# johannesulf/TabCorr

Measured on AMD Instinct MI355X. Metric: predict_calls_per_sec, higher is better.
Workload: dtype f64; 1 GPU; BASELINE configs[1]: Zheng07 predict(), synthetic auto table 50 mass bins x {cen,sat} (G=100, P=5050), 19 rp bins, n_gauss_prim=10, batch of 10000 draws per GPU per step, draws and results resident in HBM; n_tables=1, gather=none, gather_payload=ngal + xi (160 B per draw), gather_every_steps=32, lanes=4, rccl_ranks=0

## Files before the change

include/tabcorr_amd_testing.h:

```cpp
#ifndef TABCORR_AMD_TESTING_H
#define TABCORR_AMD_TESTING_H

#include "tabcorr_amd.h"

#ifdef __cplusplus
extern "C" {
#endif

int tc_debug_fastmath(int kind, int64_t n, const double* x, double* y);
int tc_debug_fastmath_device(int kind, int64_t n, const double* x, double* y);

int tc_debug_grad_operand(int n_bins, int n_r, const double* packed, double* dense);

int tc_debug_grad_lds(int kernel, int n_params, int n_bins, int n_central, int n_r, int n_dim,
                      int chi2, int64_t* bytes);

int tc_debug_leauthaud11_node_grad(const double* theta, int modulate, int64_t n,
                                   const double* mass, double* log_mstar, double* n_cen,
                                   double* dn_cen, double* n_sat, double* dn_sat);

int tc_debug_central_series(int n_gauss, double log_min, double log_max, double dist_index,
                            int64_t n, const double* log_m_min, const double* sigma,
                            double* series, double* nodes, int32_t* terms);

int tc_debug_satellite_series(int n_gauss, double log_min, double log_max, double dist_index,
                              int64_t n, const double* log_m0, const double* log_m1,
                              const double* alpha, double* series, double* nodes,
                              int32_t* terms);

int tc_plan_debug(int mode, int n_bins, const uint8_t* is_central, int n_chunks,
                  int64_t* n_entries, int32_t* entry_pair, int32_t* entry_chunk,
                  int32_t* entry_class);

int tc_debug_quad_schedule(int n_bins, int n_central, int by_type, int n_tiles, int n_rtiles,
                           int n_tables, int separate, int max_waves, int min_units,
                           int order ,
                           int* n_waves, int* n_runs, int* n_slabs, int64_t* units_min,
                           int64_t* units_max);
int tc_debug_triangle_parts(int n_rb, int n_parts, int32_t* rb0, int32_t* cb0, int32_t* count);
int tc_debug_node_groups(int n_bins, int n_central, const double* log_min,
                         const double* log_max, int32_t* begin, int32_t* member,
                         int* n_groups, int* n_central_groups);
int tc_debug_fused_form(int n_bins, int n_central, int n_r, int n_cus, int grouped,
                        int64_t n_draws, int n_gauss, unsigned flags, unsigned call,
                        const int* options, const int* measured_forms, const float* measured_us,
                        int* waves, int* draws, int* lds_bytes);
int tc_debug_pair_plan(const double* boxsize, double reach_xy, double reach_z,
                       int64_t n_points, int n_bin, int n_labels, int32_t* cells,
                       int32_t* neighbours, int32_t* labels_per_block, int32_t* n_blocks,
                       int64_t* lds_bytes);
int tc_debug_quad_emulate(int n_bins, int n_r, const double* tpcf_matrix,
                          const uint8_t* is_central, int by_type, int separate,
                          const double* densities, int64_t ldb, int64_t n_draws,
                          int max_waves, int min_units, int order, double* out);

int tc_debug_trace(tc_table* table, uint64_t* out, int64_t capacity, int64_t* n_blocks);
int tc_debug_wave_trace(tc_table* table, uint64_t* out, int64_t capacity,
                        int64_t* n_waves);
int tc_debug_resident_ticks(tc_table* table, uint64_t* out, int64_t capacity, int64_t* n_blocks);
int tc_debug_ensemble_stamps(tc_table* table, uint64_t* out);
#ifdef __cplusplus
}
// ... 4 lines not shown
```

tabcorr_amd/_lib.py:

```python

import ctypes
import os

import numpy as np

HERE = os.path.dirname(os.path.abspath(__file__))
LIBRARY = os.path.join(HERE, 'libtabcorr_hip.so')

TC_OK = 0
TC_ERR_INVALID = 1
TC_ERR_HIP = 2
TC_ERR_UNSUPPORTED = 3
TC_ERR_RCCL = 4

MODE = {'auto': 0, 'cross': 1}
DTYPE_F64 = 0
DTYPE_F32 = 1

FLAG_SEPARATE_GAL_TYPE = 1
FLAG_MODULATE_WITH_CENOCC = 2
FLAG_ASSEMBIAS = 4
FLAG_LEAUTHAUD11 = 16

UNIQUE_ID_BYTES = 128
# ... 19 lines not shown
    'tc_memcpy_d2h': [ctypes.c_void_p, ctypes.c_void_p, ctypes.c_size_t],
    'tc_host_alloc': [c_void_pp, ctypes.c_size_t],
    'tc_host_free': [ctypes.c_void_p],
    'tc_host_register': [ctypes.c_void_p, ctypes.c_size_t],
    'tc_host_unregister': [ctypes.c_void_p],
    'tc_host_is_pinned': [ctypes.c_void_p, ctypes.c_size_t, c_int_p],
    'tc_gauss_legendre': [ctypes.c_int, c_double_p, c_double_p],
    'tc_debug_fastmath': [ctypes.c_int, ctypes.c_int64, c_double_p,
                          c_double_p],
    'tc_debug_fastmath_device': [ctypes.c_int, ctypes.c_int64, c_double_p,
                                 c_double_p],
    'tc_debug_grad_operand': [ctypes.c_int, ctypes.c_int, c_double_p, c_double_p],
    'tc_debug_grad_lds': [ctypes.c_int] * 7 + [c_int64_p],
    'tc_debug_leauthaud11_node_grad': [c_double_p, ctypes.c_int, ctypes.c_int64, c_double_p,
                                       c_double_p, c_double_p, c_double_p, c_double_p,
                                       c_double_p],
    'tc_pair_indices': [ctypes.c_int, c_int32_p, c_int32_p, c_int32_p],
    'tc_spline_interpolation_matrix': [ctypes.c_int, c_double_p, c_double_p],
    'tc_spline_weights': [ctypes.c_int, c_double_p, c_double_p, ctypes.c_double, c_double_p,
                          c_double_p, c_int_p],
    'tc_plan_debug': [ctypes.c_int, ctypes.c_int, c_uint8_p, ctypes.c_int,
                      c_int64_p, c_int32_p, c_int32_p, c_int32_p],
    'tc_debug_triangle_parts': [ctypes.c_int, ctypes.c_int, c_int_p, c_int_p, c_int_p],
    'tc_debug_central_series': [ctypes.c_int, ctypes.c_double, ctypes.c_double, ctypes.c_double,
                                ctypes.c_int64, c_double_p, c_double_p, c_double_p, c_double_p,
                                c_int32_p],
    'tc_debug_satellite_series': [ctypes.c_int, ctypes.c_double, ctypes.c_double,
                                  ctypes.c_double, ctypes.c_int64, c_double_p, c_double_p,
                                  c_double_p, c_double_p, c_double_p, c_int32_p],
    'tc_debug_node_groups': [ctypes.c_int, ctypes.c_int, c_double_p, c_double_p,
                             c_int32_p, c_int32_p, c_int_p, c_int_p],
    'tc_debug_quad_schedule': [ctypes.c_int] * 10 + [c_int_p, c_int_p, c_int_p,
                                                     c_int64_p, c_int64_p],
    'tc_debug_fused_form': [ctypes.c_int] * 5 + [ctypes.c_int64, ctypes.c_int, ctypes.c_uint,
                                                 ctypes.c_uint, c_int_p, c_int_p,
                                                 c_float_p, c_int_p, c_int_p,
                                                 c_int_p],
    'tc_debug_pair_plan': [c_double_p, ctypes.c_double, ctypes.c_double, ctypes.c_int64,
                           ctypes.c_int, ctypes.c_int, c_int32_p, c_int32_p, c_int32_p,
                           c_int32_p, c_int64_p],
    'tc_debug_quad_emulate': [ctypes.c_int, ctypes.c_int, c_double_p, c_uint8_p,
                              ctypes.c_int, ctypes.c_int, c_double_p,
                              ctypes.c_int64, ctypes.c_int64, ctypes.c_int,
                              ctypes.c_int, ctypes.c_int, c_double_p],
    'tc_table_create': [
        ctypes.c_int, ctypes.c_int, ctypes.c_int, ctypes.c_int64,
# ... 239 lines not shown

_lib = None


class TabCorrHipError(RuntimeError):
    """The HIP backend failed (no device, launch error, RCCL error)."""


def load():
    global _lib
    if _lib is not None:
        return _lib
    library = os.environ.get('TABCORR_AMD_LIBRARY') or LIBRARY
    if not os.path.exists(library):
        raise TabCorrHipError(
            'libtabcorr_hip.so is missing: build it with '
            '`python -m tabcorr_amd.build` (needs hipcc). There is no CPU '
            'fallback.')
    mode = os.RTLD_NOW | os.RTLD_LOCAL | getattr(os, 'RTLD_DEEPBIND', 0)
    lib = ctypes.CDLL(library, mode=mode)
    lib.tc_last_error.restype = ctypes.c_char_p
    lib.tc_last_error.argtypes = []
    for name, argtypes in SIGNATURES.items():
        function = getattr(lib, name)
        function.restype = ctypes.c_int
        function.argtypes = argtypes
    _lib = lib
    return lib


def check(status):
    if status == TC_OK:
        return
    message = load().tc_last_error().decode(errors='replace')
    if status == TC_ERR_INVALID:
        raise ValueError(message)
    if status == TC_ERR_UNSUPPORTED:
        raise NotImplementedError(message)
    raise TabCorrHipError(message)


def as_double_p(array):
    try:
        return ctypes.byref(ctypes.c_double.from_buffer(array))
    except (TypeError, ValueError, BufferError):
        return array.ctypes.data_as(c_double_p)
# ... 36 lines not shown
```

tabcorr_amd/csrc/hostmath.cpp:

```cpp
#include "hostmath.h"
#include "fastmath.h"
#include "kernel_args.h"
#include "series.h"

#include <algorithm>
#include <atomic>
#include <cmath>
#include <cstring>
#include <map>
#include <numeric>
#include <tuple>
#include <thread>

namespace tc {

void gauss_legendre(int n, std::vector<double>& x, std::vector<double>& w) {
  x.assign(n, 0.0);
  w.assign(n, 0.0);
  const long double pi = 3.141592653589793238462643383279502884L;
  for (int i = 0; i < (n + 1) / 2; ++i) {
    long double z = cosl(pi * (i + 0.75L) / (n + 0.5L));
    long double dp = 1.0L;
    for (int iter = 0; iter < 100; ++iter) {
      long double p0 = 1.0L, p1 = z;
      for (int k = 2; k <= n; ++k) {
        long double p2 = ((2 * k - 1) * z * p1 - (k - 1) * p0) / k;
        p0 = p1;
        p1 = p2;
      }
      if (n == 0) p1 = 1.0L;
      dp = n * (z * p1 - p0) / (z * z - 1.0L);
// ... 690 lines not shown
    plan.block_begin[(size_t)block + 1] = (int32_t)plan.merges.size();
  }
  schedule.n_slabs = next_slab;
  const std::vector<int32_t> renumbered =
      number_slabs_by_group(slab_group, schedule.n_groups, schedule.group_begin);
  for (QuadRun& run : schedule.runs)
    if (run.slab >= 0) run.slab = renumbered[run.slab];
  for (QuadMerge& m : plan.merges) m.slab = renumbered[m.slab];
}

void triangle_parts(int n_rb, int n_parts, int32_t* rb0, int32_t* cb0, int32_t* count) {
  const int64_t n_units = (int64_t)n_rb * (n_rb + 1) / 2;
  for (int part = 0; part < n_parts; ++part) {
    const int64_t begin = n_units * part / n_parts, end = n_units * (part + 1) / n_parts;
    int64_t rb = (int64_t)((std::sqrt(8.0 * (double)begin + 1.0) - 1.0) / 2.0);
    while ((rb + 1) * (rb + 2) / 2 <= begin) ++rb;
    while (rb * (rb + 1) / 2 > begin) --rb;
    rb0[part] = (int32_t)rb;
    cb0[part] = (int32_t)(begin - rb * (rb + 1) / 2);
    count[part] = (int32_t)(end - begin);
  }
}

QuadTiling quad_tiling(int n_r) {
  QuadTiling tiling;
  tiling.n_rtiles = (n_r + 19) / 20;
  tiling.r_per_tile = (n_r + tiling.n_rtiles - 1) / tiling.n_rtiles;
  tiling.n_u = (tiling.r_per_tile + 3) / 4;
  return tiling;
}


int fused_dens_rows(const QuadLayout& layout) {
  int rows = 0;
  for (const QuadComp& comp : layout.comps)
    rows = std::max(rows, std::max(comp.i_bin0 + 4 * comp.n_rb, comp.j_bin0 + 4 * comp.n_cb));
  return (rows + 3) / 4 * 4;
}

int fused_lds_bytes(int dens_rows, int waves, int draws) {
  return (std::max(dens_rows * draws, fused_slot_doubles(waves, draws)) +
          fused_scratch_doubles(waves)) * 8;
}

FusedForm choose_fused_form(const FusedQuery& q) {
  const FusedForm three_kernels{};
// ... 579 lines not shown
```

tabcorr_amd/csrc/hostmath.h:

```cpp
#pragma once

#include <cstdint>
#include <string>
#include <vector>

namespace tc {

void gauss_legendre(int n, std::vector<double>& x, std::vector<double>& w);

inline int64_t packed_index(int64_t i, int64_t j) {
  return i >= j ? i * (i + 1) / 2 + j : j * (j + 1) / 2 + i;
}

bool spline_interpolation_matrix(int n, const double* xp, std::vector<double>& a);

struct Segment {
  int32_t component;
  int32_t rectangular;
  int32_t i_lo, i_hi;
  int32_t j_lo, j_hi;
  int64_t q_begin;
  int64_t n_real;
};

// ... 105 lines not shown
constexpr int kQuadUnitParts = 8;
void build_quad_schedule(const QuadLayout& layout, int n_tiles, int n_rtiles, int n_tables,
                         bool separate, int max_waves, int min_units_per_wave,
                         QuadSchedule& out, int order = kQuadTileMajor);

struct QuadMerge {
  int32_t slab;
  int32_t first_slot;
  int32_t count;
  int32_t pad;
};
struct QuadMergePlan {
  int waves_per_block = 0;
  int n_blocks = 0;
  int lds_slots = 0;
  std::vector<int32_t> block_begin;
  std::vector<QuadMerge> merges;
};
void merge_quad_schedule(const QuadLayout& layout, int n_rtiles, bool separate,
                         int waves_per_block, int max_slots, QuadSchedule& schedule,
                         QuadMergePlan& plan);

void triangle_parts(int n_rb, int n_parts, int32_t* rb0, int32_t* cb0, int32_t* count);

struct QuadTiling {
  int n_rtiles = 1;
  int r_per_tile = 0;
  int n_u = 0;
};
QuadTiling quad_tiling(int n_r);


struct AutoChoice {
  static constexpr int kSizes = 9;
  static constexpr int64_t size(int i) { return (int64_t)256 << i; }
  int form[kSizes] = {};
  float us[kSizes][3] = {};
  int form_for(int64_t n_draws) const {
    if (n_draws <= size(0)) return form[0];
    if (n_draws >= size(kSizes - 1)) return form[kSizes - 1];
    int i = 0;
    while (size(i + 1) < n_draws) ++i;
    const double w = (double)(n_draws - size(i)) / (double)(size(i + 1) - size(i));
    static const int shape[3] = {0, 64, 32};
    int best = 0;
    double best_us = (1.0 - w) * us[i][0] + w * us[i + 1][0];
// ... 102 lines not shown
```

tabcorr_amd/csrc/internal.h:

```cpp
#pragma once

#include <hip/hip_runtime.h>
#include <hip/hip_ext.h>

#include <algorithm>
#include <chrono>
#include <cmath>
#include <cstdarg>
#include <cstdio>
#include <cstdlib>
#include <cstring>
#include <functional>
#include <map>
#include <memory>
#include <string>
#include <utility>
#include <vector>

#include "../../include/tabcorr_amd.h"
#include "../../include/tabcorr_amd_testing.h"
#include "fastmath.h"
#include "grad.h"
#include "vjp.h"
#include "hostmath.h"
// ... 222 lines not shown
  int poll_done = 1;
  int quad_waves = 0;
  int quad_waves_f32 = 3;
  int quad_merge = 1;
  int quad_order = -1;
  int prio_occ = 2, prio_contract = 1, prio_finalize = 3;
  int finalize_threads = 0;
  int finalize_row_blocks = 0;
  int occ_splits = 0;
  int occ_per_cu = 4;
  int n_groups = 0, n_waves = 0, lds_min = 0, min_chunk_entries = 32;
  int k_splits = 0;
  int trace = 0;
  int autotune_after = 0;
  int sync_chunks = 0;
  int sync_form = 32;
  int sync_stagger = 10;
  int sync_direct_out = 2;
  int async_direct_in = 1;
  int async_direct_out = 2;
  int series = -1;
  int cross_defer = 1;
  int fused_defer = 2;
  int fused_sat_cap = 6;
  int cross_wide_min_draws = 4096;
  int cross_target = 160;
  int resident_aperture = 1;
  int cross_min_draws = 192;
  int fused = 1;
  int fused_min_draws = 0;
  int fused_max_draws = 30720;
  int fused_waves = 0;
  int fused_draws = 0;
  int fused_spread = 1, fused_spread_min = 8192, fused_spread_rounds = 1;
  int prio_fused = 1, prio_fused_occ = 2, prio_fused_out = 3;
  int deterministic = 0;
  int skip_occ = 0, skip_finalize = 0;
  void load() {
    fused = env_int("TC_FUSED", fused);
    fused_min_draws = env_int("TC_FUSED_MIN_DRAWS", fused_min_draws);
    fused_max_draws = env_int("TC_FUSED_MAX_DRAWS", fused_max_draws);
    prio_fused = env_int("TC_PRIO_FUSED", prio_fused);
    prio_fused_occ = env_int("TC_PRIO_FUSED_OCC", prio_fused_occ);
    prio_fused_out = env_int("TC_PRIO_FUSED_OUT", prio_fused_out);
    lanes = env_int("TC_LANES", lanes);
    pipeline = env_int("TC_PIPELINE", pipeline);
// ... 41 lines not shown
  std::vector<double> n_h, log_min, log_max, percentile, dist_index;

  void* d_table = nullptr;
  size_t table_bytes = 0;
  void* d_n_h = nullptr;
  void* d_percentile = nullptr;
  void* d_perm = nullptr;
  tc::NodeGroups node_groups;
  void* d_group_begin = nullptr;
  void* d_group_member = nullptr;
  void* d_group_n_h = nullptr;
  void* d_group_percentile = nullptr;
  bool grouped = false;
  void* d_math_table = nullptr;
  void* d_pos_ij = nullptr;
  void* d_pos_off = nullptr;
  std::vector<double> cross_host;
  tc::host::CrossFused cross_fused, cross_fused_wide;
  tc::host::GradTable grad;
  std::vector<hipEvent_t> chunk_events;
  bool quad = false;
  tc::QuadTiling quad_tiling;
  tc::host::QuadTable quad_by_type, quad_total;
  int n_cus = 256;
  int n_xcds = 8;
  tc::host::Tuning tuning;
  std::map<unsigned, AutoChoice> autotuned;
  std::map<unsigned, int> pipelined_calls;
  bool autotuning = false;
  std::map<int, tc::host::Quadrature> quadrature;
  std::map<std::pair<int, int>, std::unique_ptr<tc::host::DeviceChunking>> chunkings;
  std::map<int64_t, tc::host::DeviceChunking*> choices;

  struct Lane {
    hipStream_t stream = nullptr;
    hipEvent_t finished = nullptr;
    tc::host::DeviceBuffer nbuf, ngal2, partial;
    tc::host::DeviceBuffer nbuf32;
    tc::host::DeviceBuffer xi;
    tc::host::DeviceBuffer in_theta, out;
    tc::host::DeviceBuffer cross_counters;
    int ngal_parts = 1;
  };
  static constexpr int kMaxLanes = 8;
  Lane lanes[kMaxLanes];
  int n_lanes = 2;
// ... 258 lines not shown
```

tabcorr_amd/csrc/kernel_args.h:

```cpp
#pragma once

#include <cstdint>

#include "hostmath.h"

namespace tc {

constexpr int kLanes = 64;
constexpr unsigned kFlagSeparate = 1u;
constexpr unsigned kFlagModulate = 2u;
constexpr unsigned kFlagAssembias = 4u;
constexpr int kOccWaves = 4;
constexpr int kF32Block = 8;
constexpr int kF64Block = 8;
constexpr int kF32Tile = 32;
constexpr int kFinalizeRows = 32;
constexpr int kMaxInterpDim = 8;
constexpr int kMaxInterpAxis = 32;

struct GroupArgs {
  const int32_t* begin;
  const int32_t* member;
  const double* log_m;
  const double* m;
// ... 194 lines not shown
struct FinalizeQuadArgs {
  const void* partial;
  const int32_t* group_begin;
  const double* ngal_part;
  int n_ngal_parts;
  int n_rtiles;
  int r_per_tile;
  int rt;
  int groups_per_rtile;
  int n_comp;
  int n_r;
  int mode;
  int priority;
  int64_t ldb;
  int64_t n_draws;
  double* ngal;
  double* xi;
  const double* chi2_data;
  double* chi2;
};

constexpr int kFusedWaves = 8;
constexpr int kFusedMaxParts = 8;
constexpr int kMathTableDoubles = 2306;
constexpr int fused_slot_doubles(int waves, int draws = 64) {
  return waves * 4 * kQuadMaxU * (draws == 40 ? 40 : kQuadTile);
}
constexpr int fused_scratch_doubles(int waves) { return kMathTableDoubles + 2 * waves * kLanes; }

struct FusedArgs {
  const double* theta;
  int n_theta;
  int n_bins;
  int n_central;
  int n_gauss;
  int dens_rows;
  int part_rb0[kFusedMaxParts];
  int part_cb0[kFusedMaxParts];
  int part_count[kFusedMaxParts];
  int part_triangular[kFusedMaxParts];
  int part_n_cb[kFusedMaxParts];
  int part_i_row0[kFusedMaxParts];
  int part_j_row0[kFusedMaxParts];
  int part_unit_base[kFusedMaxParts];
  int separate;
  int n_r;
  int priority;
  int64_t n_draws;
  const double* log_m;
  const double* m;
  const double* weight;
  const double* n_h;
  const double* percentile;
  double split;
  const double* math_table;
  const void* table;
  uint32_t table_bytes;
  double* ngal;
  double* xi;
  const double* chi2_data;
  double* chi2;
  int n_groups;
  int n_central_groups;
  GroupArgs group;
  const double* series;
  const int32_t* series_thr;
  const double* sat_series;
// ... 106 lines not shown
```

tabcorr_amd/csrc/kernels.hip.h:

```cpp
#pragma once

#include <hip/hip_runtime.h>

#include <cstdint>
#include <utility>

#include "epilogue.h"
#include "fastmath.h"
#include "fused_walk.h"
#include "hostmath.h"
#include "kernel_args.h"
#include "series.h"
#include "spline.h"

#ifdef TC_DEVELOPER_KNOBS
#define TC_TRACE(pointer) ((pointer) != nullptr)
#else
#define TC_TRACE(pointer) false
#endif

namespace tc {

static_assert(sizeof(QuadRun) == 32 && sizeof(QuadCompArgs) == 32, "read as 8 x int32");

// ... 1885 lines not shown
  static_assert(!LEAUTHAUD || (NGAUSS == 0 && !ASSEMBIAS), "Leauthaud11: any n_gauss, undecorated");
  constexpr int UP = (U + 1) / 2;
  extern __shared__ __attribute__((aligned(16))) double fused_lds[];
  constexpr int kSlotDoubles = fused_slot_doubles(W, DL);
  const int region_b = a.dens_rows * DL > kSlotDoubles ? a.dens_rows * DL : kSlotDoubles;
  double* dens = fused_lds;
  double* table = fused_lds + region_b;
  double(*red)[W][kLanes] = (double(*)[W][kLanes])(table + fm::kTableDoubles);
  const fm::Consts kc = fm::make_consts();
#ifdef TC_DEVELOPER_KNOBS
  const int skip = (a.priority >> 8) & 3;
  const int n_bins_occ = (skip & 1) ? 0 : a.n_bins;
  unsigned long long* const stamps =
      ((a.priority >> 10) & 1) && a.chi2 == nullptr ? (unsigned long long*)a.chi2_data : nullptr;
  auto wave_stamp = [&](int which) {
    if (stamps != nullptr && (threadIdx.x & 63) == 0 && W == 8 && ((threadIdx.x >> 6) & 3) == 0)
      stamps[blockIdx.x * 32 + 16 + 8 * (threadIdx.x >> 8) + which] =
          __builtin_amdgcn_s_memrealtime();
  };
  auto stamp = [&](int which) {
    if (stamps != nullptr && threadIdx.x == 0)
      stamps[blockIdx.x * 32 + which] = __builtin_amdgcn_s_memrealtime();
  };
  if (skip & 1)
    for (int idx = threadIdx.x; idx < a.n_bins * DL; idx += blockDim.x) fused_lds[idx] = 1e-3;
#else
  constexpr int skip = 0;
  const int n_bins_occ = a.n_bins;
  auto stamp = [](int) {};
  auto wave_stamp = [](int) {};
#endif
  stamp(0);
  set_priority((a.priority >> 2) & 3);
  const int lane = threadIdx.x & 63;
  const int wave = __builtin_amdgcn_readfirstlane(threadIdx.x >> 6);
  const int n_gauss = NGAUSS > 0 ? NGAUSS : a.n_gauss;
  {
    typedef double __attribute__((ext_vector_type(2))) double2v;
    const int hi = fm::kTableDoubles / 2;
    const double2v* src = (const double2v*)a.math_table;
    double2v* dst = (double2v*)table;
    for (int i = threadIdx.x; i < hi; i += blockDim.x) dst[i] = src[i];
  }
  for (int idx = a.n_bins * DL + threadIdx.x; idx < a.dens_rows * DL; idx += blockDim.x)
    dens[idx] = 0.0;
  __syncthreads();
  stamp(1);

  const int draw = DL != 32 ? lane : (lane & 31);
  const int half = DL != 32 ? 0 : (lane >> 5);
  const bool live = DL != 40 || lane < 40;
  auto dens_at = [&](int row, int d) -> double& {
    return dens[DL == 40 ? dens40(row, d) : row * DL + d];
// ... 179 lines not shown
    stamp(3);
    red[0][wave][lane] = sum_cen;
    red[1][wave][lane] = sum_sat;
    __syncthreads();
    stamp(4);
    double n_cen = 0.0, n_sat = 0.0;
#pragma unroll
    for (int w = 0; w < W; ++w) {
      n_cen += red[0][w][lane];
      n_sat += red[1][w][lane];
    }
    const double total = (skip & 1) ? 1.0 : n_cen + n_sat;
    norm = total * total;
    if (wave == 0 && half == 0 && live && b0 < a.n_draws) {
      if (a.separate) {
        a.ngal[2 * b0] = n_cen;
        a.ngal[2 * b0 + 1] = n_sat;
      } else {
        a.ngal[b0] = total;
      }
    }
  }

  set_priority(a.priority & 3);
  const int c = lane & 15, kq = lane >> 4;
  double F[UP][2][2];
  constexpr int UA = DL == 40 ? (U > 3 ? 3 : U) : 1, UB = DL == 40 && U > 3 ? U - 3 : 1;
  double F40a[UA][10], F40b[UB][10];
  int slot = wave;
  if (DL == 40) {
    const int part = wave;
    const unsigned off_a = ((lane & 0x30) | ((lane & 3) << 2) | ((lane >> 2) & 3)) * 16;
    const double* dens_b = dens + (a.part_j_row0[part] + (lane >> 4)) * 40 + (lane & 3) * 10;
    const double* dens_e = dens + (a.part_i_row0[part] + (lane >> 4)) * 40 + (lane & 3) * 10;
    const __amdgpu_buffer_rsrc_t rs_t =
        __builtin_amdgcn_make_buffer_rsrc((void*)a.table, 0, a.table_bytes, kBufferFlags);
    const int rb = a.part_rb0[part], cb = a.part_cb0[part], count = a.part_count[part];
    const bool triangular = a.part_triangular[part] != 0;
    const int n_cb = a.part_n_cb[part];
    const unsigned unit_base = (unsigned)a.part_unit_base[part];
#pragma unroll
    for (int s = 0; s < UA; ++s)
#pragma unroll
      for (int g = 0; g < 10; ++g) F40a[s][g] = 0.0;
#pragma unroll
    for (int s = 0; s < UB; ++s)
#pragma unroll
      for (int g = 0; g < 10; ++g) F40b[s][g] = 0.0;
#ifdef TC_DEVELOPER_KNOBS
    const unsigned unit_bytes = ((a.priority >> 12) & 1) ? 0u : UP * 1024u;
    const unsigned first_unit = ((a.priority >> 12) & 1) ? 0u : unit_base;
#else
    constexpr unsigned unit_bytes = UP * 1024u;
    const unsigned first_unit = unit_base;
#endif
    if (!(skip & 2))
    fused_quad_pass40<0, UA>(rs_t, off_a, unit_bytes, dens_b, dens_e, rb, cb, count, triangular,
                             n_cb, first_unit, F40a);
    if (U > 3 && !(skip & 2))
      fused_quad_pass40<(U > 3 ? 3 : 0), UB>(rs_t, off_a, unit_bytes, dens_b, dens_e, rb, cb,
                                             count, triangular, n_cb, first_unit, F40b);
  } else {
    const int sub = wave / PARTS;
    const int part = (wave % PARTS + sub * (PARTS / 2)) % PARTS;
    slot = sub * PARTS + part;
    const unsigned off_a = lane * 16;
    const double* dens_b =
        dens + (a.part_j_row0[part] + kq) * DL + sub * kQuadTile + 2 * c;
    const double* dens_e = dens + a.part_i_row0[part] * DL + sub * kQuadTile + 2 * c;
    const __amdgpu_buffer_rsrc_t rs_t =
        __builtin_amdgcn_make_buffer_rsrc((void*)a.table, 0, a.table_bytes, kBufferFlags);
    const FusedPart walk = {a.part_rb0[part],        a.part_cb0[part],
                            a.part_count[part],      a.part_triangular[part],
                            a.part_n_cb[part],       (unsigned)a.part_unit_base[part]};
#pragma unroll
    for (int p = 0; p < UP; ++p) {
      F[p][0][0] = F[p][0][1] = F[p][1][0] = F[p][1][1] = 0.0;
      if (skip & 2) continue;
      if (2 * p + 1 < U)
        fused_quad_pass<2, DL>(rs_t, off_a + p * 1024, UP * 1024, dens_b, dens_e, walk, F[p]);
      else
        fused_quad_pass<1, DL>(rs_t, off_a + p * 1024, UP * 1024, dens_b, dens_e, walk, F[p]);
    }
  }
  stamp(5);
  __syncthreads();
  stamp(8);
  if (DL == 40) {
    const int q = lane >> 4;
    auto share = [&](int sub, int g) {
      return sub < UA ? F40a[sub < UA ? sub : 0][g] : F40b[sub >= UA ? sub - UA : 0][g];
    };
    double* out = dens + (wave * (4 * U) + ((lane >> 2) & 3)) * 40 + (lane & 3);
    if (((a.priority >> 11) & 1) && __builtin_amdgcn_ballot_w64(!(norm < 1e280)) == 0) {
      double select[4];
#pragma unroll
      for (int m = 0; m < 4; ++m) select[m] = (lane & 3) == m ? 1.0 : 0.0;
#pragma unroll
      for (int sub = 0; sub < U; ++sub)
#pragma unroll
        for (int t = 0; t < 3; ++t) {
          double sums = 0.0;
#pragma unroll
          for (int m = 0; m < (t < 2 ? 4 : 2); ++m)
            sums = fused_quad_rows40(select[m], share(sub, 4 * t + m), sums);
          if (t < 2 || q < 2) out[(4 * sub) * 40 + 16 * t + 4 * q] = sums;
        }
    } else {
#pragma unroll
      for (int sub = 0; sub < U; ++sub)
#pragma unroll
        for (int g = 0; g < 10; ++g) {
          const double sum = fused_quad_rows40(1.0, share(sub, g), 0.0);
          if (q == 0) out[(4 * sub) * 40 + 4 * g] = sum;
        }
    }
  } else {
    double* out = dens + (slot * (4 * U) + kq) * kQuadTile + 2 * c;
#pragma unroll
    for (int u = 0; u < U; ++u) {
      const f64x2 value = {F[u >> 1][u & 1][0], F[u >> 1][u & 1][1]};
      *(f64x2*)(out + (4 * u) * kQuadTile) = value;
    }
  }
  stamp(9);
  set_priority((a.priority >> 4) & 3);
  double(*tile)[kLanes + 1] = (double(*)[kLanes + 1])table;
  if (a.separate) {
    const bool poisoned = !(fabs(norm) <= 1.79769313486231570815e308);
    const int64_t n_valid = a.n_draws - col < DL ? a.n_draws - col : DL;
    const int sub = lane >> 5, d = lane & 31;
    for (int comp = 0; comp < 3; ++comp) {
      __syncthreads();
      constexpr int Q = PARTS / 4;
      const int p_begin = comp == 0 ? 0 : comp == 1 ? Q : 3 * Q;
      const int p_count = comp == 1 ? 2 * Q : Q;
      for (int rr = wave; rr < a.n_r && lane < DL; rr += W) {
        const double* first = dens + ((PARTS * sub + p_begin) * (4 * U) + rr) * kQuadTile + d;
        double sum = first[0];
        for (int p = 1; p < p_count; ++p) sum += first[p * (4 * U) * kQuadTile];
        tile[rr][lane] = poisoned ? __builtin_nan("") : sum / norm;
      }
      __syncthreads();
      for (int idx = threadIdx.x; idx < a.n_r * DL; idx += blockDim.x) {
        const int dd = idx / a.n_r, rr = idx % a.n_r;
// ... 1760 lines not shown
```

tabcorr_amd/csrc/launch.hip:

```cpp
#include <immintrin.h>

#include <atomic>
#include <mutex>

#include "internal.h"
#include "kernels.hip.h"
#include "series.h"

namespace tc {
namespace host {

int get_quadrature(tc_table* t, int n_gauss, Quadrature** out) {
  auto it = t->quadrature.find(n_gauss);
  if (it != t->quadrature.end()) {
    *out = &it->second;
    return TC_OK;
  }
  std::vector<double> x, w;
  tc::gauss_legendre(n_gauss, x, w);
  const int g = t->n_bins;
  std::vector<double> log_m((size_t)g * n_gauss), m((size_t)g * n_gauss),
      weight((size_t)g * n_gauss + g);
  for (int i = 0; i < g; ++i) {
    const double d_log = t->log_max[i] - t->log_min[i];
    const double exponent = t->legacy ? 0.0 : t->dist_index[i] + 1.0;
// ... 840 lines not shown
      const int first = c == 0 ? 0 : c == 1 ? quarter : 3 * quarter;
      const int pieces = c == 1 ? 2 * quarter : quarter, piece = part - first;
      const tc::QuadComp& comp = q_table.layout.comps[c];
      fa.part_triangular[part] = comp.triangular;
      fa.part_n_cb[part] = comp.n_cb;
      fa.part_i_row0[part] = comp.i_bin0;
      fa.part_j_row0[part] = comp.j_bin0;
      fa.part_unit_base[part] = (int)comp.unit_base;
      if (comp.triangular) {
        int32_t rb0[tc::kFusedMaxParts], cb0[tc::kFusedMaxParts], count[tc::kFusedMaxParts];
        tc::triangle_parts(comp.n_rb, pieces, rb0, cb0, count);
        fa.part_rb0[part] = rb0[piece];
        fa.part_cb0[part] = cb0[piece];
        fa.part_count[part] = count[piece];
      } else {
        const int64_t begin = comp.n_units * piece / pieces;
        const int64_t end = comp.n_units * (piece + 1) / pieces;
        fa.part_rb0[part] = (int)(begin / comp.n_cb);
        fa.part_cb0[part] = (int)(begin % comp.n_cb);
        fa.part_count[part] = (int)(end - begin);
      }
    }
  }
  fa.n_r = t->n_r;
  fa.priority = (t->tuning.prio_fused & 3) | ((t->tuning.prio_fused_occ & 3) << 2) |
                ((t->tuning.prio_fused_out & 3) << 4) |
                ((env_int_early("TC_FUSED_SKIP", 0) & 3) << 8) |
                (q_table.finite ? 1 << 11 : 0);
  fa.n_draws = n_draws;
  fa.n_groups = t->node_groups.n_groups;
  fa.n_central_groups = t->node_groups.n_central_groups;
  fa.group = group_args(t, *q);
  fa.series = (series_mask(t) & 1) ? (const double*)q->series : nullptr;
  fa.series_thr = (const int32_t*)q->series_thr;
  fa.sat_series = (series_mask(t) & 2) ? (const double*)q->sat_series : nullptr;
  fa.sat_series_thr = (const int32_t*)q->sat_series_thr;
  fa.log_m = (const double*)q->log_m;
  fa.m = (const double*)q->m;
  fa.weight = (const double*)q->weight;
  fa.n_h = (const double*)t->d_n_h;
  fa.percentile = (const double*)t->d_percentile;
  fa.split = 0.5;
  fa.math_table = (const double*)t->d_math_table;
  fa.table = q_table.d_table;
  fa.table_bytes =
      (uint32_t)((size_t)q_table.layout.n_units * (size_t)((t->quad_tiling.n_u + 1) / 2) * 1024);
  fa.ngal = ngal_device;
  fa.xi = xi_device;
  if (call.chi2_out != nullptr) {
    fa.chi2_data = call.chi2_data;
    fa.chi2 = call.chi2_out;
    fa.xi = nullptr;
    *chi2_written = true;
  }
  const int lds = tc::fused_lds_bytes(fa.dens_rows, waves, draws);
  const dim3 grid((unsigned)((n_draws + draws - 1) / draws)), block(64 * waves);
#ifdef TC_DEVELOPER_KNOBS
  if (fa.chi2 == nullptr && env_int_early("TC_FUSED_STAMPS", 0) != 0) {
    t->trace_blocks = ((size_t)grid.x * 32 + 5) / 6;
    status = t->trace.reserve(t->trace_blocks * 6 * sizeof(unsigned long long), stream);
    if (status != TC_OK) return status;
    fa.chi2_data = (const double*)t->trace.ptr;
    fa.priority |= 1 << 10;
  }
  if (env_int_early("TC_FUSED_SAME_UNIT", 0) != 0) fa.priority |= 1 << 12;
#endif
  hipEvent_t k0 = nullptr, k1 = nullptr;
  status = next_kernel_events(t, &k0, &k1);
  if (status != TC_OK) return status;
  const bool assembias = (flags & TC_FLAG_ASSEMBIAS) != 0;
  const bool modulate = (flags & TC_FLAG_MODULATE_WITH_CENOCC) != 0;
  const bool sat_defer = t->tuning.fused_defer != 0 && !assembias && !modulate &&
                         !(flags & TC_FLAG_LEAUTHAUD11) && n_gauss == 10 && draws != 32 &&
                         waves == 8 && t->n_bins <= 256 &&
                         !(t->grouped && n_gauss == 10) && t->tuning.series != 0 &&
                         q->sat_series != nullptr && q->sat_records != nullptr;
  if (sat_defer) fa.sat_series = (const double*)q->sat_series;
  fa.sat_records = (const double*)q->sat_records;
  fa.cen_records = (const double*)q->cen_records;
  const bool cen_defer = sat_defer && t->tuning.fused_defer >= 2 && (series_mask(t) & 1) != 0 &&
                         q->cen_records != nullptr;
  fa.sat_cap = t->tuning.fused_sat_cap;
  tc::host::FusedInstance instance{};
  instance.n_gauss = n_gauss == 10 ? 10 : 0;
  instance.assembias = assembias;
  instance.modulate = modulate;
  instance.leauthaud = (flags & TC_FLAG_LEAUTHAUD11) != 0;
  instance.waves = waves;
// ... 1142 lines not shown
```

tabcorr_amd/csrc/runtime.cpp:

```cpp
#include <dlfcn.h>
#include <pthread.h>

#include <atomic>
#include <condition_variable>
#include <mutex>
#include <new>
#include <thread>
#include <vector>

#include "grad_leauthaud11.h"
#include "internal.h"
#include "series.h"

namespace tc {
namespace host {

namespace {
thread_local std::string g_last_error;
}

namespace {
struct Roctx {
  int (*push)(const char*) = nullptr;
  int (*pop)() = nullptr;
// ... 707 lines not shown
        const int64_t column =
            mode == TC_MODE_AUTO
                ? tc::packed_index(plan.perm[plan.pos_i[q]], plan.perm[plan.pos_j[q]])
                : plan.perm[plan.pos_j[q]];
        if (column != plan.column[q])
          return fail(TC_ERR_INVALID, "bin pair mismatch at position %d", q);
        if (e >= plan.n_entries) return fail(TC_ERR_INVALID, "too many entries");
        entry_pair[e] = (int32_t)column;
        entry_chunk[e] = c;
        entry_class[e] = chunk.component;
        ++e;
      }
    }
  }
  for (int64_t q = 0; q < plan.n_positions; ++q)
    if (!seen[q]) return fail(TC_ERR_INVALID, "position %lld not covered", (long long)q);
  if (e != plan.n_entries) return fail(TC_ERR_INVALID, "entries missing");
  return TC_OK;
}

int tc_debug_triangle_parts(int n_rb, int n_parts, int32_t* rb0, int32_t* cb0, int32_t* count) {
  TC_CHECK(n_rb >= 1 && n_parts >= 1 && rb0 && cb0 && count, "invalid argument");
  tc::triangle_parts(n_rb, n_parts, rb0, cb0, count);
  return TC_OK;
}

int tc_debug_fused_form(int n_bins, int n_central, int n_r, int n_cus, int grouped,
                        int64_t n_draws, int n_gauss, unsigned flags, unsigned call,
                        const int* options, const int* measured_forms, const float* measured_us,
                        int* waves, int* draws, int* lds_bytes) {
  TC_CHECK(n_bins >= 1 && n_central >= 0 && n_central <= n_bins && n_r >= 1 && n_cus >= 1 &&
               options && waves && draws && lds_bytes && (!measured_forms == !measured_us),
           "invalid arguments");
  const tc::QuadTiling tiling = tc::quad_tiling(n_r);
  tc::QuadLayout by_type, total;
  tc::build_quad_layout(n_bins, n_central, true, by_type);
  const bool fusable = tiling.n_rtiles == 1 && n_r <= 20 && n_bins <= 248;
  const bool has_total = (n_central % 4 != 0 && n_central < n_bins) || fusable;
  if (has_total) tc::build_quad_layout(n_bins, n_central, false, total);
  tc::FusedQuery q;
  q.n_bins = n_bins;
  q.n_u = tiling.n_u;
  q.n_cus = n_cus;
  q.grouped = grouped != 0;
  q.servable = has_total && tiling.n_rtiles == 1 && n_r <= 20;
  q.units_total = total.n_units;
// ... 144 lines not shown
```

tabcorr_amd/csrc/table.cpp:

```cpp
#include <cmath>

#include "internal.h"

using namespace tc::host;

extern "C" {

int tc_table_create(int mode, int n_bins, int n_r, int64_t n_pairs,
                    const void* tpcf_matrix, int matrix_dtype, const double* n_h,
                    const double* log_min, const double* log_max,
                    const double* percentile, const double* dist_index,
                    const uint8_t* is_central, int compute_dtype, tc_table** out) {
  TC_CHECK(out != nullptr, "table output pointer is NULL");
  *out = nullptr;
  TC_CHECK(mode == TC_MODE_AUTO || mode == TC_MODE_CROSS, "invalid mode %d", mode);
  TC_CHECK(n_bins >= 1 && n_bins < (1 << 20), "invalid number of bins %d", n_bins);
  TC_CHECK(n_r >= 1, "invalid number of correlation function bins %d", n_r);
  const int64_t expect =
      mode == TC_MODE_AUTO ? (int64_t)n_bins * (n_bins + 1) / 2 : n_bins;
  TC_CHECK(n_pairs == expect,
           "tpcf_matrix has %lld columns but %d bins in mode '%s' need %lld",
           (long long)n_pairs, n_bins, mode == TC_MODE_AUTO ? "auto" : "cross",
           (long long)expect);
  TC_CHECK(n_pairs < (1LL << 31), "too many pair columns");
// ... 1620 lines not shown
  } else if (key == "resident_min_walkers") {
    TC_CHECK(value >= 2 && value <= 256, "resident_min_walkers must be in [2, 256]");
    t->resident.min_walkers = value;
  } else if (key == "resident_wait_us") {
    TC_CHECK(value >= 1 && value <= 1000000, "resident_wait_us must be in [1, 1000000]");
    const int status = resident_stop(t);
    if (status != TC_OK) return status;
    t->resident.wait_us = value;
  } else if (key == "resident_aperture") {
    TC_CHECK(value == 0 || value == 1, "resident_aperture must be 0 or 1");
    const int status = resident_stop(t);
    if (status != TC_OK) return status;
    t->tuning.resident_aperture = value;
    t->resident.ens_grid = 0;
    t->resident.single_aperture_decided = false;
  } else if (key == "cross_min_draws") {
    TC_CHECK(value >= 1, "cross_min_draws must be positive");
    t->tuning.cross_min_draws = value;
  } else if (key == "cross_defer") {
    t->tuning.cross_defer = value != 0;
  } else if (key == "fused_defer") {
    TC_CHECK(value >= 0 && value <= 2, "fused_defer must be 0, 1 or 2");
    t->tuning.fused_defer = value;
  } else if (key == "fused_sat_cap") {
    TC_CHECK(value >= 0 && value <= 6, "fused_sat_cap must be in [0, 6]");
    t->tuning.fused_sat_cap = value;
  } else if (key == "cross_wide_min_draws") {
    TC_CHECK(value >= 0, "cross_wide_min_draws must not be negative");
    t->tuning.cross_wide_min_draws = value;
  } else if (key == "cross_target") {
    TC_CHECK(value >= 1 && value <= 4096, "cross_target must be in [1, 4096]");
    t->tuning.cross_target = value;
  } else if (key == "series") {
    TC_CHECK(value >= -1 && value <= 3, "series must be -1 .. 3");
    t->tuning.series = value;
  } else if (key == "grouped") {
    t->grouped = value != 0 && t->node_groups.largest > 1;
  } else if (key == "lanes") {
    TC_CHECK(value >= 1 && value <= (int)tc_table::kMaxLanes, "lanes must be in [1, %d]",
             (int)tc_table::kMaxLanes);
    for (tc_table::Lane& lane : t->lanes)
      if (lane.stream) TC_HIP(hipStreamSynchronize(lane.stream));
    for (int l = 0; l < value; ++l) {
      if (t->lanes[l].stream != nullptr) continue;
      TC_HIP(hipStreamCreateWithFlags(&t->lanes[l].stream, hipStreamNonBlocking));
      TC_HIP(hipEventCreateWithFlags(&t->lanes[l].finished, hipEventDisableTiming));
// ... 207 lines not shown
```

Before: 279.1 million calls/s.

## Balance fused quad waves by assigning parts per pass from a host cost model

New measurement: 281.5 million calls/s, median of 6. Within noise of the previous version (+0.8%).

```diff
diff --git a/include/tabcorr_amd_testing.h b/include/tabcorr_amd_testing.h
--- a/include/tabcorr_amd_testing.h
+++ b/include/tabcorr_amd_testing.h
@@ -38,6 +38,10 @@
                            int* n_waves, int* n_runs, int* n_slabs, int64_t* units_min,
                            int64_t* units_max);
 int tc_debug_triangle_parts(int n_rb, int n_parts, int32_t* rb0, int32_t* cb0, int32_t* count);
+int tc_debug_fused_shares(int n_parts, const int32_t* rb0, const int32_t* cb0,
+                          const int32_t* count, const int32_t* triangular, const int32_t* n_cb,
+                          int n_u, int waves, int by_cost, uint8_t* share, int32_t* rows,
+                          int64_t* wave_cost, int64_t* constants);
 int tc_debug_node_groups(int n_bins, int n_central, const double* log_min,
                          const double* log_max, int32_t* begin, int32_t* member,
                          int* n_groups, int* n_central_groups);
diff --git a/tabcorr_amd/_lib.py b/tabcorr_amd/_lib.py
--- a/tabcorr_amd/_lib.py
+++ b/tabcorr_amd/_lib.py
@@ -65,6 +65,8 @@
     'tc_plan_debug': [ctypes.c_int, ctypes.c_int, c_uint8_p, ctypes.c_int,
                       c_int64_p, c_int32_p, c_int32_p, c_int32_p],
     'tc_debug_triangle_parts': [ctypes.c_int, ctypes.c_int, c_int_p, c_int_p, c_int_p],
+    'tc_debug_fused_shares': [ctypes.c_int] + [c_int32_p] * 5 + [ctypes.c_int] * 3 +
+                             [c_uint8_p, c_int32_p, c_int64_p, c_int64_p],
     'tc_debug_central_series': [ctypes.c_int, ctypes.c_double, ctypes.c_double, ctypes.c_double,
                                 ctypes.c_int64, c_double_p, c_double_p, c_double_p, c_double_p,
                                 c_int32_p],
@@ -350,6 +352,9 @@
     lib.tc_last_error.restype = ctypes.c_char_p
     lib.tc_last_error.argtypes = []
     for name, argtypes in SIGNATURES.items():
+        if (library != LIBRARY and name.startswith('tc_debug_')
+                and not hasattr(lib, name)):
+            continue
         function = getattr(lib, name)
         function.restype = ctypes.c_int
         function.argtypes = argtypes
diff --git a/tabcorr_amd/csrc/hostmath.cpp b/tabcorr_amd/csrc/hostmath.cpp
--- a/tabcorr_amd/csrc/hostmath.cpp
+++ b/tabcorr_amd/csrc/hostmath.cpp
@@ -7,6 +7,7 @@
 #include <atomic>
 #include <cmath>
 #include <cstring>
+#include <functional>
 #include <map>
 #include <numeric>
 #include <tuple>
@@ -743,6 +744,139 @@
   }
 }
 
+const int64_t kFusedShareUnit[2] = {128, 205};
+const int64_t kFusedShareRow[2] = {175, 366};
+const int64_t kFusedShareAge = 1120;
+
+int fused_part_rows(const FusedShareParts& parts, int part) {
+  int rb = parts.rb0[part], cb = parts.cb0[part], rows = 0;
+  for (int64_t left = parts.count[part]; left > 0; ++rows, ++rb, cb = 0) {
+    const int length = parts.triangular[part] ? rb + 1 : parts.n_cb[part];
+    if (length <= cb) return rows;
+    left -= length - cb;
+  }
+  return rows;
+}
+
+int64_t fused_job_cost(const FusedShareParts& parts, int part, int sub_tiles) {
+  const int k = sub_tiles > 1 ? 1 : 0;
+  return std::max<int64_t>(parts.count[part], 0) * kFusedShareUnit[k] +
+         (int64_t)fused_part_rows(parts, part) * kFusedShareRow[k];
+}
+
+namespace {
+
+struct ShareSearch {
+  int n = 0, passes = 0;
+  int64_t job[kFusedSharePasses][kFusedShareParts] = {};
+  int64_t age[kFusedShareParts] = {};
+  void key(const unsigned char (*perm)[kFusedShareParts], int64_t* out) const {
+    for (int i = 0; i < n; ++i) {
+      int64_t sum = 0;
+      for (int p = 0; p < passes; ++p) sum += job[p][perm[p][i]];
+      out[i] = sum * age[i];
+    }
+    std::sort(out, out + n, std::greater<int64_t>());
+  }
+  bool better(const int64_t* a, const int64_t* b) const {
+    return std::lexicographical_compare(a, a + n, b, b + n);
+  }
+};
+
+}
+
+static int share_passes(int n_u) { return std::min(std::max((n_u + 1) / 2, 1), kFusedSharePasses); }
+static int share_sub_tiles(int n_u, int pass) { return 2 * pass + 1 < n_u ? 2 : 1; }
+
+void fused_shares(const FusedShareParts& parts, int n_u, int waves, bool by_cost,
+                  unsigned char (*share)[kFusedSharePasses]) {
+  const int n = std::min(std::max(parts.n_parts, 1), kFusedShareParts);
+  const int tiles = std::max(std::min(waves, kFusedShareWaves) / n, 1);
+  for (int w = 0; w < kFusedShareWaves; ++w)
+    for (int p = 0; p < kFusedSharePasses; ++p) share[w][p] = 0;
+  ShareSearch search;
+  search.n = n;
+  search.passes = share_passes(n_u);
+  for (int p = 0; p < search.passes; ++p)
+    for (int part = 0; part < n; ++part)
+      search.job[p][part] = fused_job_cost(parts, part, share_sub_tiles(n_u, p));
+  for (int i = 0; i < n; ++i) search.age[i] = tiles == 1 && i >= n / 2 ? kFusedShareAge : 1000;
+  unsigned char best[kFusedSharePasses][kFusedShareParts];
+  for (int p = 0; p < kFusedSharePasses; ++p)
+    for (int i = 0; i < n; ++i) best[p][i] = (unsigned char)i;
+  if (by_cost) {
+    int64_t best_key[kFusedShareParts], key[kFusedShareParts];
+    search.key(best, best_key);
+    unsigned char perm[kFusedSharePasses][kFusedShareParts];
+    auto take_if_better = [&]() {
+      search.key(perm, key);
+      if (!search.better(key, best_key)) return false;
+      std::copy(key, key + n, best_key);
+      std::copy(&perm[0][0], &perm[0][0] + kFusedSharePasses * kFusedShareParts, &best[0][0]);
+      return true;
+    };
+    std::copy(&best[0][0], &best[0][0] + kFusedSharePasses * kFusedShareParts, &perm[0][0]);
+    if (n <= 4) {
+      std::function<void(int)> pass = [&](int p) {
+        if (p == search.passes) {
+          take_if_better();
+          return;
+        }
+        for (int i = 0; i < n; ++i) perm[p][i] = (unsigned char)i;
+        do pass(p + 1);
+        while (std::next_permutation(perm[p], perm[p] + n));
+      };
+      pass(0);
+    } else {
+      int64_t load[kFusedShareParts] = {};
+      for (int p = 0; p < search.passes; ++p) {
+        int order[kFusedShareParts];
+        bool taken[kFusedShareParts] = {};
+        for (int i = 0; i < n; ++i) order[i] = i;
+        std::stable_sort(order, order + n,
+                         [&](int a, int b) { return search.job[p][a] > search.job[p][b]; });
+        for (int k = 0; k < n; ++k) {
+          int wave = -1;
+          for (int i = 0; i < n; ++i)
+            if (!taken[i] && (wave < 0 || load[i] * search.age[i] < load[wave] * search.age[wave]))
+              wave = i;
+          taken[wave] = true;
+          perm[p][wave] = (unsigned char)order[k];
+          load[wave] += search.job[p][order[k]];
+        }
+      }
+      take_if_better();
+      std::copy(&best[0][0], &best[0][0] + kFusedSharePasses * kFusedShareParts, &perm[0][0]);
+      for (bool moved = true; moved;) {
+        moved = false;
+        for (int p = 0; p < search.passes; ++p)
+          for (int i = 0; i < n; ++i)
+            for (int j = i + 1; j < n; ++j) {
+              std::swap(perm[p][i], perm[p][j]);
+              if (take_if_better()) moved = true;
+              else std::swap(perm[p][i], perm[p][j]);
+            }
+      }
+    }
+  }
+  for (int tile = 0; tile < tiles; ++tile)
+    for (int i = 0; i < n; ++i)
+      for (int p = 0; p < search.passes; ++p)
+        share[tile * n + i][p] = best[p][(i + tile * (n / 2)) % n];
+}
+
+void fused_share_costs(const FusedShareParts& parts, int n_u, int waves,
+                       const unsigned char (*share)[kFusedSharePasses], int64_t* cost) {
+  const int n = std::min(std::max(parts.n_parts, 1), kFusedShareParts);
+  const int tiles = std::max(std::min(waves, kFusedShareWaves) / n, 1);
+  for (int w = 0; w < tiles * n; ++w) {
+    int64_t sum = 0;
+    for (int p = 0; p < share_passes(n_u); ++p)
+      sum += fused_job_cost(parts, share[w][p] % n, share_sub_tiles(n_u, p));
+    cost[w] = sum * (w >= tiles * n / 2 ? kFusedShareAge : 1000);
+  }
+}
+
 QuadTiling quad_tiling(int n_r) {
   QuadTiling tiling;
   tiling.n_rtiles = (n_r + 19) / 20;
diff --git a/tabcorr_amd/csrc/hostmath.h b/tabcorr_amd/csrc/hostmath.h
--- a/tabcorr_amd/csrc/hostmath.h
+++ b/tabcorr_amd/csrc/hostmath.h
@@ -151,6 +151,20 @@
                          QuadMergePlan& plan);
 
 void triangle_parts(int n_rb, int n_parts, int32_t* rb0, int32_t* cb0, int32_t* count);
+
+constexpr int kFusedShareParts = 8, kFusedShareWaves = 16, kFusedSharePasses = 3;
+struct FusedShareParts {
+  int n_parts = 0;
+  int32_t rb0[kFusedShareParts] = {}, cb0[kFusedShareParts] = {}, count[kFusedShareParts] = {};
+  int32_t triangular[kFusedShareParts] = {}, n_cb[kFusedShareParts] = {};
+};
+int fused_part_rows(const FusedShareParts& parts, int part);
+int64_t fused_job_cost(const FusedShareParts& parts, int part, int sub_tiles);
+void fused_shares(const FusedShareParts& parts, int n_u, int waves, bool by_cost,
+                  unsigned char (*share)[kFusedSharePasses]);
+void fused_share_costs(const FusedShareParts& parts, int n_u, int waves,
+                       const unsigned char (*share)[kFusedSharePasses], int64_t* cost);
+extern const int64_t kFusedShareUnit[2], kFusedShareRow[2], kFusedShareAge;
 
 struct QuadTiling {
   int n_rtiles = 1;
diff --git a/tabcorr_amd/csrc/internal.h b/tabcorr_amd/csrc/internal.h
--- a/tabcorr_amd/csrc/internal.h
+++ b/tabcorr_amd/csrc/internal.h
@@ -268,6 +268,7 @@
   int series = -1;
   int cross_defer = 1;
   int fused_defer = 2;
+  int fused_shares = 1;
   int fused_sat_cap = 6;
   int cross_wide_min_draws = 4096;
   int cross_target = 160;
@@ -355,6 +356,12 @@
   bool quad = false;
   tc::QuadTiling quad_tiling;
   tc::host::QuadTable quad_by_type, quad_total;
+  struct FusedShares {
+    bool valid = false;
+    int waves = 0, by_cost = 0;
+    tc::FusedShareParts parts;
+    unsigned char share[tc::kFusedShareWaves][tc::kFusedSharePasses] = {};
+  } fused_shares[2];
   int n_cus = 256;
   int n_xcds = 8;
   tc::host::Tuning tuning;
diff --git a/tabcorr_amd/csrc/kernel_args.h b/tabcorr_amd/csrc/kernel_args.h
--- a/tabcorr_amd/csrc/kernel_args.h
+++ b/tabcorr_amd/csrc/kernel_args.h
@@ -240,6 +240,8 @@
 
 constexpr int kFusedWaves = 8;
 constexpr int kFusedMaxParts = 8;
+static_assert(kFusedShareParts == kFusedMaxParts && kFusedShareWaves == 2 * kFusedMaxParts &&
+                  kFusedSharePasses == (kQuadMaxU + 1) / 2, "hostmath.h: fused_shares");
 constexpr int kMathTableDoubles = 2306;
 constexpr int fused_slot_doubles(int waves, int draws = 64) {
   return waves * 4 * kQuadMaxU * (draws == 40 ? 40 : kQuadTile);
@@ -261,6 +263,7 @@
   int part_i_row0[kFusedMaxParts];
   int part_j_row0[kFusedMaxParts];
   int part_unit_base[kFusedMaxParts];
+  uint32_t share[kFusedShareWaves];
   int separate;
   int n_r;
   int priority;
diff --git a/tabcorr_amd/csrc/kernels.hip.h b/tabcorr_amd/csrc/kernels.hip.h
--- a/tabcorr_amd/csrc/kernels.hip.h
+++ b/tabcorr_amd/csrc/kernels.hip.h
@@ -1931,6 +1931,12 @@
     if (stamps != nullptr && threadIdx.x == 0)
       stamps[blockIdx.x * 32 + which] = __builtin_amdgcn_s_memrealtime();
   };
+  auto wave_end_stamp = [&]() {
+    if (stamps != nullptr && (threadIdx.x & 63) == 0 && W == 8) {
+      const int w = threadIdx.x >> 6;
+      stamps[blockIdx.x * 32 + (w < 5 ? 11 + w : 16 + w)] = __builtin_amdgcn_s_memrealtime();
+    }
+  };
   if (skip & 1)
     for (int idx = threadIdx.x; idx < a.n_bins * DL; idx += blockDim.x) fused_lds[idx] = 1e-3;
 #else
@@ -1938,6 +1944,7 @@
   const int n_bins_occ = a.n_bins;
   auto stamp = [](int) {};
   auto wave_stamp = [](int) {};
+  auto wave_end_stamp = []() {};
 #endif
   stamp(0);
   set_priority((a.priority >> 2) & 3);
@@ -2163,12 +2170,16 @@
     }
   }
 
+#ifdef TC_DEVELOPER_KNOBS
+  set_priority(((a.priority >> 13) & 1) && threadIdx.x >= 32 * W ? 1 : (a.priority & 3));
+#else
   set_priority(a.priority & 3);
+#endif
   const int c = lane & 15, kq = lane >> 4;
   double F[UP][2][2];
   constexpr int UA = DL == 40 ? (U > 3 ? 3 : U) : 1, UB = DL == 40 && U > 3 ? U - 3 : 1;
   double F40a[UA][10], F40b[UB][10];
-  int slot = wave;
+  int part_of[UP] = {};
   if (DL == 40) {
     const int part = wave;
     const unsigned off_a = ((lane & 0x30) | ((lane & 3) << 2) | ((lane >> 2) & 3)) * 16;
@@ -2203,19 +2214,20 @@
                                              count, triangular, n_cb, first_unit, F40b);
   } else {
     const int sub = wave / PARTS;
-    const int part = (wave % PARTS + sub * (PARTS / 2)) % PARTS;
-    slot = sub * PARTS + part;
     const unsigned off_a = lane * 16;
-    const double* dens_b =
-        dens + (a.part_j_row0[part] + kq) * DL + sub * kQuadTile + 2 * c;
-    const double* dens_e = dens + a.part_i_row0[part] * DL + sub * kQuadTile + 2 * c;
     const __amdgpu_buffer_rsrc_t rs_t =
         __builtin_amdgcn_make_buffer_rsrc((void*)a.table, 0, a.table_bytes, kBufferFlags);
-    const FusedPart walk = {a.part_rb0[part],        a.part_cb0[part],
-                            a.part_count[part],      a.part_triangular[part],
-                            a.part_n_cb[part],       (unsigned)a.part_unit_base[part]};
+    const unsigned shares = a.share[wave];
 #pragma unroll
     for (int p = 0; p < UP; ++p) {
+      const int part = (shares >> (8 * p)) & (kFusedMaxParts - 1);
+      part_of[p] = part;
+      const double* dens_b =
+          dens + (a.part_j_row0[part] + kq) * DL + sub * kQuadTile + 2 * c;
+      const double* dens_e = dens + a.part_i_row0[part] * DL + sub * kQuadTile + 2 * c;
+      const FusedPart walk = {a.part_rb0[part],        a.part_cb0[part],
+                              a.part_count[part],      a.part_triangular[part],
+                              a.part_n_cb[part],       (unsigned)a.part_unit_base[part]};
       F[p][0][0] = F[p][0][1] = F[p][1][0] = F[p][1][1] = 0.0;
       if (skip & 2) continue;
       if (2 * p + 1 < U)
@@ -2224,6 +2236,7 @@
         fused_quad_pass<1, DL>(rs_t, off_a + p * 1024, UP * 1024, dens_b, dens_e, walk, F[p]);
     }
   }
+  wave_end_stamp();
   stamp(5);
   __syncthreads();
   stamp(8);
@@ -2257,11 +2270,12 @@
         }
     }
   } else {
-    double* out = dens + (slot * (4 * U) + kq) * kQuadTile + 2 * c;
+    double* out = dens + kq * kQuadTile + 2 * c;
 #pragma unroll
     for (int u = 0; u < U; ++u) {
+      const int slot = wave / PARTS * PARTS + part_of[u >> 1];
       const f64x2 value = {F[u >> 1][u & 1][0], F[u >> 1][u & 1][1]};
-      *(f64x2*)(out + (4 * u) * kQuadTile) = value;
+      *(f64x2*)(out + (slot * (4 * U) + 4 * u) * kQuadTile) = value;
     }
   }
   stamp(9);
diff --git a/tabcorr_amd/csrc/launch.hip b/tabcorr_amd/csrc/launch.hip
--- a/tabcorr_amd/csrc/launch.hip
+++ b/tabcorr_amd/csrc/launch.hip
@@ -1,6 +1,7 @@
 #include <immintrin.h>
 
 #include <atomic>
+#include <cstring>
 #include <mutex>
 
 #include "internal.h"
@@ -887,6 +888,32 @@
       }
     }
   }
+  if (draws != 40) {
+    tc::FusedShareParts parts;
+    parts.n_parts = n_parts;
+    for (int part = 0; part < n_parts; ++part) {
+      parts.rb0[part] = fa.part_rb0[part];
+      parts.cb0[part] = fa.part_cb0[part];
+      parts.count[part] = fa.part_count[part];
+      parts.triangular[part] = fa.part_triangular[part];
+      parts.n_cb[part] = fa.part_n_cb[part];
+    }
+    tc_table::FusedShares& kept = t->fused_shares[separate ? 1 : 0];
+    const int by_cost = t->tuning.fused_shares != 0 ? 1 : 0;
+    if (!kept.valid || kept.waves != waves || kept.by_cost != by_cost ||
+        std::memcmp(&kept.parts, &parts, sizeof(parts)) != 0) {
+      tc::fused_shares(parts, t->quad_tiling.n_u, waves, by_cost != 0, kept.share);
+      kept.parts = parts;
+      kept.waves = waves;
+      kept.by_cost = by_cost;
+      kept.valid = true;
+    }
+    for (int w = 0; w < tc::kFusedShareWaves; ++w) {
+      fa.share[w] = 0;
+      for (int p = 0; p < tc::kFusedSharePasses; ++p)
+        fa.share[w] |= (uint32_t)kept.share[w][p] << (8 * p);
+    }
+  }
   fa.n_r = t->n_r;
   fa.priority = (t->tuning.prio_fused & 3) | ((t->tuning.prio_fused_occ & 3) << 2) |
                 ((t->tuning.prio_fused_out & 3) << 4) |
@@ -929,6 +956,7 @@
     fa.priority |= 1 << 10;
   }
   if (env_int_early("TC_FUSED_SAME_UNIT", 0) != 0) fa.priority |= 1 << 12;
+  if (env_int_early("TC_FUSED_PRIO_YOUNG", 0) != 0) fa.priority |= 1 << 13;
 #endif
   hipEvent_t k0 = nullptr, k1 = nullptr;
   status = next_kernel_events(t, &k0, &k1);
diff --git a/tabcorr_amd/csrc/runtime.cpp b/tabcorr_amd/csrc/runtime.cpp
--- a/tabcorr_amd/csrc/runtime.cpp
+++ b/tabcorr_amd/csrc/runtime.cpp
@@ -753,6 +753,42 @@
 int tc_debug_triangle_parts(int n_rb, int n_parts, int32_t* rb0, int32_t* cb0, int32_t* count) {
   TC_CHECK(n_rb >= 1 && n_parts >= 1 && rb0 && cb0 && count, "invalid argument");
   tc::triangle_parts(n_rb, n_parts, rb0, cb0, count);
+  return TC_OK;
+}
+
+int tc_debug_fused_shares(int n_parts, const int32_t* rb0, const int32_t* cb0,
+                          const int32_t* count, const int32_t* triangular, const int32_t* n_cb,
+                          int n_u, int waves, int by_cost, uint8_t* share, int32_t* rows,
+                          int64_t* wave_cost, int64_t* constants) {
+  TC_CHECK((n_parts == 4 || n_parts == 8) && rb0 && cb0 && count && triangular && n_cb && share,
+           "invalid argument");
+  TC_CHECK(n_u >= 1 && n_u <= tc::kQuadMaxU && (waves == n_parts || waves == 2 * n_parts),
+           "invalid form");
+  tc::FusedShareParts parts;
+  parts.n_parts = n_parts;
+  for (int part = 0; part < n_parts; ++part) {
+    TC_CHECK(rb0[part] >= 0 && cb0[part] >= 0 && count[part] >= 0 && n_cb[part] >= 1 &&
+                 cb0[part] < (triangular[part] ? rb0[part] + 1 : n_cb[part]),
+             "invalid part");
+    parts.rb0[part] = rb0[part];
+    parts.cb0[part] = cb0[part];
+    parts.count[part] = count[part];
+    parts.triangular[part] = triangular[part];
+    parts.n_cb[part] = n_cb[part];
+  }
+  unsigned char table[tc::kFusedShareWaves][tc::kFusedSharePasses];
+  tc::fused_shares(parts, n_u, waves, by_cost != 0, table);
+  std::memcpy(share, table, sizeof(table));
+  if (rows)
+    for (int part = 0; part < n_parts; ++part) rows[part] = tc::fused_part_rows(parts, part);
+  if (wave_cost) tc::fused_share_costs(parts, n_u, waves, table, wave_cost);
+  if (constants) {
+    constants[0] = tc::kFusedShareUnit[0];
+    constants[1] = tc::kFusedShareUnit[1];
+    constants[2] = tc::kFusedShareRow[0];
+    constants[3] = tc::kFusedShareRow[1];
+    constants[4] = tc::kFusedShareAge;
+  }
   return TC_OK;
 }
 
diff --git a/tabcorr_amd/csrc/table.cpp b/tabcorr_amd/csrc/table.cpp
--- a/tabcorr_amd/csrc/table.cpp
+++ b/tabcorr_amd/csrc/table.cpp
@@ -1666,6 +1666,9 @@
   } else if (key == "fused_defer") {
     TC_CHECK(value >= 0 && value <= 2, "fused_defer must be 0, 1 or 2");
     t->tuning.fused_defer = value;
+  } else if (key == "fused_shares") {
+    TC_CHECK(value == 0 || value == 1, "fused_shares must be 0 or 1");
+    t->tuning.fused_shares = value;
   } else if (key == "fused_sat_cap") {
     TC_CHECK(value >= 0 && value <= 6, "fused_sat_cap must be in [0, 6]");
     t->tuning.fused_sat_cap = value;
```
